# SYSTRAN/faster-whisper

Hardware: AMD Instinct MI355X
Metric: audio-sec/sec (RTF) large-v3 fp16 beam=5 batch=16 (higher is better)
Workload: dtype f16

## Files before the change

faster_whisper_amd/csrc/dec_kernels.hip:

```cpp
#include "common.h"
#include "dec_kernels.h"
#include <stdlib.h>
#include <atomic>
#include <type_traits>

namespace fwd {
static std::atomic<int> g_self_attn_form{0};
static std::atomic<int> g_forms_epoch{0};
static std::atomic<int> g_cross_regs{0};
}

__device__ __forceinline__ size_t frag_off(int row, int k, int KS) {
  return ((size_t)((row >> 4) * KS + (k >> 5)) * 64 + ((k >> 3) & 3) * 16 + (row & 15)) * 8 + (k & 7);
}

__global__ void dec_embed_kernel(const int* __restrict__ tok, const half_t* __restrict__ emb,
                                 const half_t* __restrict__ pos_emb, half_t* __restrict__ x,
                                 half_t* __restrict__ xfrag, int d, const int* __restrict__ d_step, int pos_fixed,
                                 int P, int blk_n) {
  const int r = blockIdx.x;
  const int pos = blk_n > 0 ? pos_fixed + r % blk_n : (pos_fixed >= 0 ? pos_fixed : P - 1 + *d_step);
  const half2_t* e = reinterpret_cast<const half2_t*>(emb + (size_t)tok[r] * d);
  const half2_t* pe = reinterpret_cast<const half2_t*>(pos_emb + (size_t)pos * d);
  half2_t* xo = reinterpret_cast<half2_t*>(x + (size_t)r * d);
// ... 718 lines not shown
    if (LNF) {
      float sa, sb;
      if (SPLIT) {
        sa = xst[a][i][0]; sb = xst[a][i][1];
      } else {
        sa = rs[a]; sb = rq[a];
        sa += __shfl_xor(sa, 16, 64); sa += __shfl_xor(sa, 32, 64);
        sb += __shfl_xor(sb, 16, 64); sb += __shfl_xor(sb, 32, 64);
      }
      mu = sa / (float)K;
      rstd = rsqrtf(fmaxf(sb / (float)K - mu * mu, 0.f) + 1e-5f);
    }
    const int row = (rt0 + a) * 16 + i;
    if (rt0 + a >= n_rt || row >= R) continue;
    const float sx = I8 ? x_scale[row] : 1.f;
    const bool pair_ok = (ldo & 1) == 0;
#pragma unroll
    for (int b = 0; b < NT; ++b) {
      if (ct0 + b >= n_ct) continue;
      const int n = (ct0 + b) * 16 + 4 * g;
      float t4[4];
#pragma unroll
      for (int e = 0; e < 4; ++e) {
        float tv = I8 ? (float)acci[a][b][e] * sx * kws[b][e] : accf[a][b][e];
        if (LNF) tv = rstd * (tv - mu * ks1[b][e]) + kcf[b][e];
        else if (bias) tv += (float)kb[b][e];
        t4[e] = tv;
      }
      if (F32 && pair_ok) {
        float* o = reinterpret_cast<float*>(outv) + (size_t)row * ldo + n;
        if (n + 1 < N) *reinterpret_cast<floatx2*>(o) = floatx2{t4[0], t4[1]};
        else if (n < N) o[0] = t4[0];
        if (n + 3 < N) *reinterpret_cast<floatx2*>(o + 2) = floatx2{t4[2], t4[3]};
        else if (n + 2 < N) o[2] = t4[2];
        continue;
      }
#pragma unroll
      for (int e = 0; e < 4; ++e) {
        if (n + e >= N) continue;
        if (F32) reinterpret_cast<float*>(outv)[(size_t)row * ldo + n + e] = t4[e];
        else reinterpret_cast<half_t*>(outv)[(size_t)row * ldo + n + e] = (half_t)t4[e];
      }
    }
  }
}

#define SA_MAX_CTX 448
static __device__ __forceinline__ float sum8_dpp(float v) {
  v += __builtin_bit_cast(float, __builtin_amdgcn_update_dpp(0, __builtin_bit_cast(int, v), 0xB1, 0xF, 0xF, true));
  v += __builtin_bit_cast(float, __builtin_amdgcn_update_dpp(0, __builtin_bit_cast(int, v), 0x4E, 0xF, 0xF, true));
  v += __builtin_bit_cast(float, __builtin_amdgcn_update_dpp(0, __builtin_bit_cast(int, v), 0x141, 0xF, 0xF, true));
  return v;
}
__global__ __launch_bounds__(1024) __attribute__((amdgpu_waves_per_eu(8, 8))) void dec_self_attn_kernel(const half_t* __restrict__ qkv, int d, half_t* __restrict__ kc,
                                                             half_t* __restrict__ vc, int n_ctx, int cache_ctx,
                                                             int H, const uint8_t* __restrict__ kvidx2, int Kbeam, int kmul,
                                                             half_t* __restrict__ out, const int* __restrict__ d_step,
                                                             int pos_fixed, int P, int R_total, int frag) {
  extern __shared__ float sa_smem[];
  const int lane = threadIdx.x & 63;
  const int wave = __builtin_amdgcn_readfirstlane(threadIdx.x >> 6);
  float* sp = sa_smem + (size_t)wave * 2 * n_ctx;
  int* ssrc = reinterpret_cast<int*>(sp + n_ctx);
  const int h = blockIdx.x, c = blockIdx.y;
  const int r = c * kmul + wave, kb = wave;
  const int step = *d_step;
  const int pos = pos_fixed >= 0 ? pos_fixed : P - 1 + step;
  const int slot = c * Kbeam + kb;
  const int cur = (pos_fixed >= 0) ? 0 : (step & 1);
  const uint8_t* kvidx = kvidx2 + ((size_t)cur * R_total + slot) * n_ctx;
  const half_t* qr = qkv + (size_t)r * 3 * d + h * 64;
  const size_t head_stride = (size_t)cache_ctx * 64;
  const size_t slot_stride = (size_t)H * head_stride;
  const int pg = lane >> 3, cc = lane & 7;
  const half8_t q8 = *reinterpret_cast<const half8_t*>(qr + cc * 8);
  const half8_t kn8 = *reinterpret_cast<const half8_t*>(qr + d + cc * 8);
  const half8_t vn8 = *reinterpret_cast<const half8_t*>(qr + 2 * d + cc * 8);
  float q[8];
#pragma unroll
  for (int e = 0; e < 8; ++e) q[e] = (float)q8[e] * 0.125f;
  if (pg == 0) {
    *reinterpret_cast<half8_t*>(kc + slot * slot_stride + h * head_stride + (size_t)pos * 64 + cc * 8) = kn8;
    *reinterpret_cast<half8_t*>(vc + slot * slot_stride + h * head_stride + (size_t)pos * 64 + cc * 8) = vn8;
  }
  auto dot8 = [&](const half8_t& k) {
    float sacc = 0.f;
#pragma unroll
    for (int e = 0; e < 8; ++e) sacc += q[e] * (float)k[e];
    return sum8_dpp(sacc);
  };
  const float s_new = dot8(kn8);
  float mx = s_new;
  const half_t* kbase = kc + h * head_stride + cc * 8;
  for (int p0 = 0; p0 < pos; p0 += 32) {
    half8_t kv[4];
    int src[4];
#pragma unroll
    for (int j = 0; j < 4; ++j) {
      const int p = p0 + 8 * j + pg;
      const int pc = p < pos ? p : pos - 1;
      src[j] = c * Kbeam + kvidx[pc];
      kv[j] = *reinterpret_cast<const half8_t*>(kbase + src[j] * slot_stride + (size_t)pc * 64);
    }
#pragma unroll
    for (int j = 0; j < 4; ++j) {
      const int p = p0 + 8 * j + pg;
      const float sc = dot8(kv[j]);
      if (p < pos) {
        if (cc == 0) { sp[p] = sc; ssrc[p] = src[j]; }
        mx = fmaxf(mx, sc);
      }
    }
  }
  mx = wave_max(mx);
  __builtin_amdgcn_wave_barrier();
  float sum = 0.f;
  for (int p = lane; p < pos; p += 64) {
    const float e = __expf(sp[p] - mx);
    sp[p] = e;
    sum += e;
  }
  const float e_new = __expf(s_new - mx);
  sum = wave_sum(sum) + e_new;
  __builtin_amdgcn_wave_barrier();
  float acc[8];
#pragma unroll
  for (int e = 0; e < 8; ++e) acc[e] = 0.f;
  const half_t* vb = vc + h * head_stride + cc * 8;
#pragma unroll 4
  for (int p = pg; p < pos; p += 8) {
    const half8_t vv = *reinterpret_cast<const half8_t*>(vb + ssrc[p] * slot_stride + (size_t)p * 64);
    const float w = sp[p];
#pragma unroll
    for (int e = 0; e < 8; ++e) acc[e] += w * (float)vv[e];
  }
#pragma unroll
  for (int e = 0; e < 8; ++e) {
    float a = acc[e];
    a += __shfl_xor(a, 8, 64);
    a += __shfl_xor(a, 16, 64);
    a += __shfl_xor(a, 32, 64);
    acc[e] = a;
  }
  if (pg == 0) {
    const float inv = 1.f / sum;
    half8_t o;
#pragma unroll
    for (int e = 0; e < 8; ++e) o[e] = (half_t)((acc[e] + e_new * (float)vn8[e]) * inv);
    half_t* dst = frag ? out + frag_off(r, h * 64 + cc * 8, d >> 5) : out + (size_t)r * d + h * 64 + cc * 8;
    *reinterpret_cast<half8_t*>(dst) = o;
  }
}

template <int U, bool PIPE, int MAXT, bool PB = false>
__global__ __launch_bounds__(MAXT) void dec_self_attn2_kernel(const half_t* __restrict__ qkv, int d, half_t* __restrict__ kc,
                                                             half_t* __restrict__ vc, int n_ctx, int cache_ctx,
                                                             int H, const uint8_t* __restrict__ kvidx2, int Kbeam, int kmul,
                                                             half_t* __restrict__ out, const int* __restrict__ d_step,
                                                             int pos_fixed, int P, int R_total, int frag) {
  extern __shared__ float sa_smem[];
  constexpr int NB = 4 * U;
  const int lane = threadIdx.x & 63;
  const int wave = __builtin_amdgcn_readfirstlane(threadIdx.x >> 6);
  float* sp = sa_smem + (size_t)wave * 2 * n_ctx;
  int* ssrc = reinterpret_cast<int*>(sp + n_ctx);
  const int h = blockIdx.x, c = blockIdx.y;
  const int r = c * kmul + wave, kb = PB ? 0 : wave;
  const int step = PB ? 0 : *d_step;
  const int pos = PB ? pos_fixed + wave : (pos_fixed >= 0 ? pos_fixed : P - 1 + step);
  const int slot = c * Kbeam + kb;
  const int cur = (pos_fixed >= 0) ? 0 : (step & 1);
  const uint8_t* kvidx = kvidx2 + ((size_t)cur * R_total + slot) * n_ctx;
  const half_t* qr = qkv + (size_t)r * 3 * d + h * 64;
  const size_t head_stride = (size_t)cache_ctx * 64;
  const size_t slot_stride = (size_t)H * head_stride;
  const int pg = lane >> 3, cc = lane & 7;
  for (int p4 = 4 * lane; p4 < pos; p4 += 256) {
    const unsigned w = PB ? 0u : *reinterpret_cast<const unsigned*>(kvidx + p4);
    intx4 s4;
    s4[0] = c * Kbeam + (int)(w & 0xffu); s4[1] = c * Kbeam + (int)((w >> 8) & 0xffu);
    s4[2] = c * Kbeam + (int)((w >> 16) & 0xffu); s4[3] = c * Kbeam + (int)(w >> 24);
    *reinterpret_cast<intx4*>(ssrc + p4) = s4;
  }
  const half8_t q8 = *reinterpret_cast<const half8_t*>(qr + cc * 8);
  const half8_t kn8 = *reinterpret_cast<const half8_t*>(qr + d + cc * 8);
  const half8_t vn8 = *reinterpret_cast<const half8_t*>(qr + 2 * d + cc * 8);
  float q[8];
#pragma unroll
  for (int e = 0; e < 8; ++e) q[e] = (float)q8[e] * 0.125f;
  if (pg == 0) {
    *reinterpret_cast<half8_t*>(kc + slot * slot_stride + h * head_stride + (size_t)pos * 64 + cc * 8) = kn8;
    *reinterpret_cast<half8_t*>(vc + slot * slot_stride + h * head_stride + (size_t)pos * 64 + cc * 8) = vn8;
  }
  auto dot8 = [&](const half8_t& k) {
    float sacc = 0.f;
#pragma unroll
    for (int e = 0; e < 8; ++e) sacc = __builtin_fmaf(q[e], (float)k[e], sacc);
    return sum8_dpp(sacc);
  };
  const float s_new = dot8(kn8);
  float mx = s_new;
  __builtin_amdgcn_wave_barrier();
  const char* kbase = reinterpret_cast<const char*>(kc + h * head_stride);
  const char* vbase = reinterpret_cast<const char*>(vc + h * head_stride);
  const unsigned slot_bytes = (unsigned)(slot_stride * sizeof(half_t));
  struct Batch { half8_t row[NB]; };
  auto fetch = [&](Batch& b, const char* base, int p0, const half_t* sib) {
#pragma unroll
    for (int j = 0; j < NB; ++j) {
      const int p = p0 + 8 * j + pg;
      const int pc = p < pos ? p : pos - 1;
      const unsigned off = (unsigned)ssrc[pc] * slot_bytes + (unsigned)(pc * 128 + cc * 16);
      if (PB && pc >= pos_fixed)
        b.row[j] = *reinterpret_cast<const half8_t*>(sib + (size_t)(pc - pos_fixed) * 3 * d + cc * 8);
      else
        b.row[j] = *reinterpret_cast<const half8_t*>(base + off);
    }
  };
  const half_t* ksib = qkv + (size_t)c * kmul * 3 * d + d + h * 64;
  const half_t* vsib = ksib + d;
  auto score = [&](const Batch& b, int p0) {
#pragma unroll
    for (int j = 0; j < NB; ++j) {
      const int p = p0 + 8 * j + pg;
      const float sc = dot8(b.row[j]);
      if (p < pos) {
        if (cc == 0) sp[p] = sc;
        mx = fmaxf(mx, sc);
      }
    }
  };
  Batch b0, b1;
  if (pos > 0) {
    fetch(b0, kbase, 0, ksib);
    for (int p0 = 0; p0 < pos; p0 += 16 * NB) {
      if (PIPE) {
        fetch(b1, kbase, p0 + 8 * NB, ksib);
        score(b0, p0);
        fetch(b0, kbase, p0 + 16 * NB, ksib);
        score(b1, p0 + 8 * NB);
      } else {
        score(b0, p0);
        if (p0 + 8 * NB < pos) {
          fetch(b0, kbase, p0 + 8 * NB, ksib);
          score(b0, p0 + 8 * NB);
          if (p0 + 16 * NB < pos) fetch(b0, kbase, p0 + 16 * NB, ksib);
        }
      }
    }
    fetch(b0, vbase, 0, vsib);
  }
  mx = wave_max_v(mx);
  __builtin_amdgcn_wave_barrier();
  float sum = 0.f;
  for (int p = lane; p < pos; p += 64) {
    const float e = __expf(sp[p] - mx);
    sp[p] = e;
    sum += e;
  }
  const float e_new = __expf(s_new - mx);
  sum = wave_sum_v(sum) + e_new;
  __builtin_amdgcn_wave_barrier();
  float acc[8];
#pragma unroll
  for (int e = 0; e < 8; ++e) acc[e] = 0.f;
  auto accum = [&](const Batch& b, int p0) {
#pragma unroll
    for (int j = 0; j < NB; ++j) {
      const int p = p0 + 8 * j + pg;
      if (p < pos) {
        const float w = sp[p];
#pragma unroll
        for (int e = 0; e < 8; ++e) acc[e] = __builtin_fmaf(w, (float)b.row[j][e], acc[e]);
      }
    }
  };
  for (int p0 = 0; p0 < pos; p0 += 16 * NB) {
    if (PIPE) {
      fetch(b1, vbase, p0 + 8 * NB, vsib);
      accum(b0, p0);
      fetch(b0, vbase, p0 + 16 * NB, vsib);
      accum(b1, p0 + 8 * NB);
    } else {
      accum(b0, p0);
      if (p0 + 8 * NB < pos) {
        fetch(b0, vbase, p0 + 8 * NB, vsib);
        accum(b0, p0 + 8 * NB);
        if (p0 + 16 * NB < pos) fetch(b0, vbase, p0 + 16 * NB, vsib);
      }
    }
  }
#pragma unroll
  for (int e = 0; e < 8; ++e) acc[e] = sum_x8_x16_x32_v(acc[e]);
  if (pg == 0) {
    const float inv = 1.f / sum;
    half8_t o;
#pragma unroll
    for (int e = 0; e < 8; ++e) o[e] = (half_t)((acc[e] + e_new * (float)vn8[e]) * inv);
    half_t* dst = frag ? out + frag_off(r, h * 64 + cc * 8, d >> 5) : out + (size_t)r * d + h * 64 + cc * 8;
    *reinterpret_cast<half8_t*>(dst) = o;
  }
}

template <int CA_WAVES, bool NTL, int MINW = 1>
__global__ __launch_bounds__(CA_WAVES * 64, MINW) void dec_cross_attn_kernel(const half_t* __restrict__ qx, int d,
                                                             const half_t* __restrict__ ck,
                                                             const half_t* __restrict__ cvt, int T, int kvp,
                                                             int kmul, half_t* __restrict__ out,
                                                             const int* __restrict__ done, int kv_div, int frag,
                                                             const int* __restrict__ slot_map) {
  __shared__ float sm[CA_WAVES][16], sl[CA_WAVES][16];
  __shared__ float so[CA_WAVES][16][65];
  const int h = blockIdx.x, c = blockIdx.y;
  if (done && done[c]) return;
  const int tid = threadIdx.x, lane = tid & 63, wave = tid >> 6;
  const int j = lane & 15, g = lane >> 4;
  const int ce = slot_map[c / kv_div];
  const half_t* kbase = ck + ((size_t)ce * (d >> 6) + h) * kvp * 64 + lane * 8;
  const half_t* vbase = cvt + ((size_t)ce * (d >> 6) + h) * kvp * 64 + lane * 8;
  half8_t qf[2];
  {
    if (j < kmul) {
      const half_t* qp = qx + (size_t)(c * kmul + j) * d + h * 64 + g * 8;
#pragma unroll
      for (int s = 0; s < 2; ++s) {
        half8_t v = *reinterpret_cast<const half8_t*>(qp + s * 32);
#pragma unroll
        for (int e = 0; e < 8; ++e) v[e] = v[e] * (half_t)0.125f;
        qf[s] = v;
      }
    } else {
      qf[0] = half8_t{0, 0, 0, 0, 0, 0, 0, 0};
      qf[1] = qf[0];
    }
  }
  floatx4 o[4];
#pragma unroll
  for (int dt = 0; dt < 4; ++dt) o[dt] = floatx4{0, 0, 0, 0};
  float m_run = -1.0e30f, l_run = 0.f;
  const float LOG2E = 1.4426950408889634f;
  const int ngroups = (T + 31) >> 5;
  auto load_kv = [&](int gi, half8_t (&kf)[4], half8_t (&vf)[4]) {
    const half_t* kp = kbase + (size_t)gi * 2048;
    const half_t* vp = vbase + (size_t)gi * 2048;
#pragma unroll
    for (int q = 0; q < 4; ++q)
      kf[q] = NTL ? __builtin_nontemporal_load(reinterpret_cast<const half8_t*>(kp + q * 512))
                  : *reinterpret_cast<const half8_t*>(kp + q * 512);
#pragma unroll
    for (int dt = 0; dt < 4; ++dt)
      vf[dt] = NTL ? __builtin_nontemporal_load(reinterpret_cast<const half8_t*>(vp + dt * 512))
                   : *reinterpret_cast<const half8_t*>(vp + dt * 512);
  };
  half8_t kcur[4], vcur[4], knxt[4], vnxt[4];
  if (wave < ngroups) load_kv(wave, kcur, vcur);
  for (int gi = wave; gi < ngroups; gi += CA_WAVES) {
    const int base = gi * 32;
    const bool has_next = (gi + CA_WAVES) < ngroups;
    if (has_next) load_kv(gi + CA_WAVES, knxt, vnxt);
    floatx4 s0 = {0, 0, 0, 0}, s1 = {0, 0, 0, 0};
    s0 = __builtin_amdgcn_mfma_f32_16x16x32_f16(kcur[0], qf[0], s0, 0, 0, 0);
    s0 = __builtin_amdgcn_mfma_f32_16x16x32_f16(kcur[1], qf[1], s0, 0, 0, 0);
    s1 = __builtin_amdgcn_mfma_f32_16x16x32_f16(kcur[2], qf[0], s1, 0, 0, 0);
    s1 = __builtin_amdgcn_mfma_f32_16x16x32_f16(kcur[3], qf[1], s1, 0, 0, 0);
    float sc[8];
    float mx = -1.0e30f;
#pragma unroll
    for (int e = 0; e < 8; ++e) {
      float v = (e < 4 ? s0[e] : s1[e - 4]) * LOG2E;
      if (base + 8 * g + e >= T) v = -1.0e30f;
      sc[e] = v;
      mx = fmaxf(mx, v);
    }
    mx = pair16_max(mx);
    mx = pair32_max(mx);
    const float m_new = fmaxf(m_run, mx);
    const float alpha = __builtin_amdgcn_exp2f(m_run - m_new);
    m_run = m_new;
    half8_t pf;
    float psum = 0.f;
#pragma unroll
    for (int e = 0; e < 8; ++e) {
      const float pv = __builtin_amdgcn_exp2f(sc[e] - m_new);
      psum += pv;
      pf[e] = (half_t)pv;
    }
    l_run = l_run * alpha + psum;
#pragma unroll
    for (int dt = 0; dt < 4; ++dt) {
#pragma unroll
      for (int e = 0; e < 4; ++e) o[dt][e] *= alpha;
      o[dt] = __builtin_amdgcn_mfma_f32_16x16x32_f16(vcur[dt], pf, o[dt], 0, 0, 0);
    }
    if (has_next) {
#pragma unroll
      for (int q = 0; q < 4; ++q) { kcur[q] = knxt[q]; vcur[q] = vnxt[q]; }
    }
  }
  l_run = pair16_sum(l_run);
  l_run = pair32_sum(l_run);
  if (g == 0) { sm[wave][j] = m_run; sl[wave][j] = l_run; }
#pragma unroll
  for (int dt = 0; dt < 4; ++dt)
#pragma unroll
    for (int e = 0; e < 4; ++e) so[wave][j][dt * 16 + 4 * g + e] = o[dt][e];
  __syncthreads();
  for (int idx = tid; idx < kmul * 64; idx += CA_WAVES * 64) {
    const int qq = idx >> 6, dh = idx & 63;
    float M = sm[0][qq];
#pragma unroll
    for (int w = 1; w < CA_WAVES; ++w) M = fmaxf(M, sm[w][qq]);
    float Lsum = 0.f, O = 0.f;
#pragma unroll
    for (int w = 0; w < CA_WAVES; ++w) {
      const float f = __builtin_amdgcn_exp2f(sm[w][qq] - M);
      Lsum += sl[w][qq] * f;
      O += so[w][qq][dh] * f;
    }
    const int orow = c * kmul + qq;
    half_t* dst = frag ? out + frag_off(orow, h * 64 + dh, d >> 5) : out + (size_t)orow * d + h * 64 + dh;
    *dst = (half_t)(O / Lsum);
  }
}

__global__ __launch_bounds__(1024) void dec_nospeech_kernel(const float* __restrict__ logits, int V, int row_mul,
                                                            int no_speech_id, float* __restrict__ out) {
  __shared__ float red[32];
  const int b = blockIdx.x;
  const float* lg = logits + (size_t)b * row_mul * V;
  float mx = -3.0e38f;
  for (int v = threadIdx.x; v < V; v += blockDim.x) mx = fmaxf(mx, lg[v]);
  mx = wave_max(mx);
  if ((threadIdx.x & 63) == 0) red[threadIdx.x >> 6] = mx;
  __syncthreads();
  float m2 = -3.0e38f;
  for (int i = 0; i < (int)(blockDim.x >> 6); ++i) m2 = fmaxf(m2, red[i]);
  __syncthreads();
  float s = 0.f;
  for (int v = threadIdx.x; v < V; v += blockDim.x) s += __expf(lg[v] - m2);
  s = wave_sum(s);
  if ((threadIdx.x & 63) == 0) red[threadIdx.x >> 6] = s;
  __syncthreads();
  if (threadIdx.x == 0) {
    float tot = 0.f;
// ... 477 lines not shown
    case 0: frag_variant<4, 2, 2, 5>(st, lnf, xf, Wf, bias, s1, cf, out, R, N, K); break;
    case 1: frag_variant<8, 2, 2, 5>(st, lnf, xf, Wf, bias, s1, cf, out, R, N, K); break;
    case 2: frag_variant<8, 4, 2, 3>(st, lnf, xf, Wf, bias, s1, cf, out, R, N, K); break;
    case 3: frag_variant<8, 4, 2, 4>(st, lnf, xf, Wf, bias, s1, cf, out, R, N, K); break;
    case 4: frag_variant<8, 4, 4, 2>(st, lnf, xf, Wf, bias, s1, cf, out, R, N, K); break;
    case 5: frag_variant<8, 4, 4, 3>(st, lnf, xf, Wf, bias, s1, cf, out, R, N, K); break;
    case 6: frag_variant<4, 4, 2, 3>(st, lnf, xf, Wf, bias, s1, cf, out, R, N, K); break;
    case 7: frag_variant<8, 2, 4, 3>(st, lnf, xf, Wf, bias, s1, cf, out, R, N, K); break;
    case 8: frag_variant<8, 8, 2, 2>(st, lnf, xf, Wf, bias, s1, cf, out, R, N, K); break;
    case 9: frag_variant<4, 4, 4, 2>(st, lnf, xf, Wf, bias, s1, cf, out, R, N, K); break;
    case 23: frag_variant<4, 1, 1, 10>(st, lnf, xf, Wf, bias, s1, cf, out, R, N, K); break;
    case 24: frag_variant<8, 1, 1, 10>(st, lnf, xf, Wf, bias, s1, cf, out, R, N, K); break;
    case 25: frag_variant<4, 1, 2, 6>(st, lnf, xf, Wf, bias, s1, cf, out, R, N, K); break;
    case 26: frag_variant<8, 1, 2, 6>(st, lnf, xf, Wf, bias, s1, cf, out, R, N, K); break;
    case 21: frag_variant<4, 4, 4, 5>(st, lnf, xf, Wf, bias, s1, cf, out, R, N, K); break;
    case 22: frag_variant<8, 4, 4, 5>(st, lnf, xf, Wf, bias, s1, cf, out, R, N, K); break;
    case 10: case 11: case 12:
      return launch_dec_gemm_big(st, variant - 10, xf, Wf, lnf ? nullptr : bias, lnf ? s1 : nullptr, lnf ? cf : nullptr,
                                 nullptr, 0, out, N, nullptr, R, N, K, 0);
    default: return -1;
  }
  return 0;
}

static int dec_linear_role(int N, int K) { return N == 3 * K ? 0 : (N >= 2560 ? 2 : (K >= 2560 ? 3 : 1)); }
struct DecBigRule { int rows; int cfg; };
static const DecBigRule DEC_BIG_RULES[4][2] = {
     {{640, 2}, {1280, 0}},
     {{1088, 1}, {1 << 30, 1}},
     {{512, 2}, {1280, 0}},
     {{832, 1}, {1 << 30, 1}},
};
static int dec_big_cfg_for(int R, int N, int K) {
  const DecBigRule* r = DEC_BIG_RULES[dec_linear_role(N, K)];
  if (R >= r[1].rows) return r[1].cfg;
  if (R >= r[0].rows) return r[0].cfg;
  return -1;
}
#define DEC_BIG_MIN_ROWS_I8 1024
int dec_big_min_rows_of(int role, int compute_type) {
  if (compute_type == 1) return DEC_BIG_MIN_ROWS_I8;
  if (role >= 0 && role < 4) return DEC_BIG_RULES[role][0].rows;
  int lo = DEC_BIG_RULES[0][0].rows;
  for (int k = 1; k < 4; ++k) lo = DEC_BIG_RULES[k][0].rows < lo ? DEC_BIG_RULES[k][0].rows : lo;
  return lo;
}

static bool skinny_one_tile(int R, int N) { return R <= 16 || (R <= 96 && N <= 1280); }

int launch_dec_gemm_frag(hipStream_t st, const half_t* xf, const half_t* Wf, const half_t* bias, const float* s1,
                         const float* cf, const half_t* res, int ldr, half_t* out, int ldo, half_t* out_frag, int R,
                         int N, int K, int act) {
  const int cfg = dec_big_cfg_for(R, N, K);
  if (cfg >= 0 &&
      launch_dec_gemm_big(st, cfg, xf, Wf, bias, s1, cf, res, ldr, out, ldo, out_frag, R, N, K, act) == 0)
    return 0;
  return launch_dec_gemm_skinny(st, xf, Wf, bias, s1, cf, res, ldr, out, ldo, out_frag, R, N, K, act);
}

int dec_big_min_rows() { return dec_big_min_rows_of(-1, 0); }

int launch_dec_gemm_skinny(hipStream_t st, const half_t* xf, const half_t* Wf, const half_t* bias, const float* s1,
                           const float* cf, const half_t* res, int ldr, half_t* out, int ldo, half_t* out_frag, int R,
                           int N, int K, int act) {
  if (K % 32 != 0 || N % 32 != 0 || R < 1) return -1;
  const int waves = K >= 2560 ? 8 : 4;
  const bool one_tile = skinny_one_tile(R, N);
  if (one_tile) {
    if (s1) frag_go<true, 1, 1, 10>(st, waves, xf, Wf, bias, s1, cf, res, ldr, out, ldo, out_frag, R, N, K, act);
    else frag_go<false, 1, 1, 10>(st, waves, xf, Wf, bias, s1, cf, res, ldr, out, ldo, out_frag, R, N, K, act);
    return 0;
  }
  if (s1) frag_go<true, 2, 2>(st, waves, xf, Wf, bias, s1, cf, res, ldr, out, ldo, out_frag, R, N, K, act);
  else frag_go<false, 2, 2>(st, waves, xf, Wf, bias, s1, cf, res, ldr, out, ldo, out_frag, R, N, K, act);
  return 0;
}

int launch_dec_gemm_skinny_tiles(hipStream_t st, int tiles, const half_t* xf, const half_t* Wf, const half_t* bias,
                                 const float* s1, const float* cf, const half_t* res, int ldr, half_t* out, int ldo,
                                 half_t* out_frag, int R, int N, int K, int act) {
  if (K % 32 != 0 || N % 32 != 0 || R < 1) return -1;
  const int waves = K >= 2560 ? 8 : 4;
  if (tiles == 1) {
    if (s1) frag_go<true, 1, 1, 10>(st, waves, xf, Wf, bias, s1, cf, res, ldr, out, ldo, out_frag, R, N, K, act);
    else frag_go<false, 1, 1, 10>(st, waves, xf, Wf, bias, s1, cf, res, ldr, out, ldo, out_frag, R, N, K, act);
  } else if (tiles == 2) {
    if (s1) frag_go<true, 2, 2>(st, waves, xf, Wf, bias, s1, cf, res, ldr, out, ldo, out_frag, R, N, K, act);
    else frag_go<false, 2, 2>(st, waves, xf, Wf, bias, s1, cf, res, ldr, out, ldo, out_frag, R, N, K, act);
  } else {
    return -1;
  }
  return 0;
}

int launch_dec_gemm_frag_i8(hipStream_t st, const int8_t* xq, const float* x_scale, const int8_t* Wq,
                            const float* w_scale, const half_t* bias, const half_t* res, int ldr, half_t* out, int ldo,
                            int R, int N, int K, int act) {
  if (K % 64 != 0 || N % 32 != 0 || R < 1 || !x_scale || !w_scale) return -1;
  if (R >= DEC_BIG_MIN_ROWS_I8 && N % 64 == 0) {
    const dim3 g4(N / 64, ((R + 15) / 16 + 3) / 4);
    if (K >= 2560)
      dec_gemm_frag_i8_kernel<8, 4, 4, 3><<<g4, 512, 0, st>>>(xq, x_scale, Wq, w_scale, bias, res, ldr, out, ldo, R, N, K, act);
    else
      dec_gemm_frag_i8_kernel<4, 4, 4, 5><<<g4, 256, 0, st>>>(xq, x_scale, Wq, w_scale, bias, res, ldr, out, ldo, R, N, K, act);
    return 0;
  }
  const dim3 grid(N / 32, ((R + 15) / 16 + 1) / 2);
  if (K >= 2560)
    dec_gemm_frag_i8_kernel<8, 2, 2><<<grid, 512, 0, st>>>(xq, x_scale, Wq, w_scale, bias, res, ldr, out, ldo, R, N, K, act);
  else
    dec_gemm_frag_i8_kernel<4, 2, 2><<<grid, 256, 0, st>>>(xq, x_scale, Wq, w_scale, bias, res, ldr, out, ldo, R, N, K, act);
  return 0;
}

template <bool I8, bool LNF, int RT>
static void wave_go(hipStream_t st, const void* xf, const float* x_scale, const void* Wf, const float* w_scale,
                    const float* s1, const float* cf, float* out, int ldo, int R, int N, int K) {
  constexpr int NT = 2, WM = 1, WN = 4;
  const int n_rt = (R + 15) / 16, n_ct = (N + 15) / 16;
  const int n_cg = ((n_ct + NT * WN - 1) / (NT * WN) + 7) & ~7;
  const int n_rg = (n_rt + RT * WM - 1) / (RT * WM);
  dec_gemm_wave_kernel<I8, LNF, true, RT, NT, WM, WN><<<n_cg * n_rg, WM * WN * 64, 0, st>>>(
      xf, x_scale, Wf, w_scale, nullptr, s1, cf, out, ldo, R, N, K, n_rg);
}

int launch_dec_logits(hipStream_t st, bool i8, const void* xf, const float* x_scale, const void* Wf,
                      const float* w_scale, const float* s1, const float* cf, float* out, int ldo, int R, int N, int K) {
  if (K % (i8 ? 64 : 32) != 0 || R < 1) return -1;
  if (i8 ? (!x_scale || !w_scale) : ((s1 == nullptr) != (cf == nullptr))) return -1;
  const int n_rt = (R + 15) / 16;
#define WG(RT)                                                                                   \
  do {                                                                                           \
    if (i8) wave_go<true, false, RT>(st, xf, x_scale, Wf, w_scale, s1, cf, out, ldo, R, N, K);   \
    else if (s1) wave_go<false, true, RT>(st, xf, x_scale, Wf, w_scale, s1, cf, out, ldo, R, N, K); \
    else wave_go<false, false, RT>(st, xf, x_scale, Wf, w_scale, s1, cf, out, ldo, R, N, K);     \
  } while (0)
  if (n_rt == 1) WG(1);
  else if (n_rt == 2) WG(2);
  else if (n_rt == 3) WG(3);
  else if (n_rt == 4) WG(4);
  else WG(5);
#undef WG
  return 0;
}

bool self_attn_block_ok(int n_ctx, int cache_ctx, int d, int R_total) {
  return (n_ctx & 3) == 0 && (size_t)R_total * cache_ctx * d * sizeof(half_t) < ((size_t)1 << 32);
}

void launch_self_attn(hipStream_t st, const half_t* qkv, int d, half_t* kc, half_t* vc, int n_ctx, int cache_ctx, int H,
                      const uint8_t* kvidx2, int Kbeam, int kmul, half_t* out, int rows, const int* d_step,
                      int pos_fixed, int P, int R_total, int frag, int blk_n) {
  if (blk_n > 0) {
    dec_self_attn2_kernel<1, true, 1024, true><<<dim3(H, rows / blk_n), blk_n * 64, (size_t)blk_n * 2 * n_ctx * sizeof(float), st>>>(
        qkv, d, kc, vc, n_ctx, cache_ctx, H, kvidx2, Kbeam, blk_n, out, d_step, pos_fixed, P, R_total, frag);
    return;
  }
  const dim3 grid(H, rows / kmul);
  const size_t lds = (size_t)kmul * 2 * n_ctx * sizeof(float);
  int form = g_self_attn_form.load(std::memory_order_relaxed);
  if ((n_ctx & 3) != 0 || (size_t)R_total * cache_ctx * d * sizeof(half_t) >= ((size_t)1 << 32)) form = 1;
  if (form == 0) form = (kmul <= 8 && (int)(grid.x * grid.y) <= 768) ? 2 : 3;
  if (form == 2 && kmul > 8) form = 3;
#define SA_ARGS qkv, d, kc, vc, n_ctx, cache_ctx, H, kvidx2, Kbeam, kmul, out, d_step, pos_fixed, P, R_total, frag
  if (form == 1) dec_self_attn_kernel<<<grid, kmul * 64, lds, st>>>(SA_ARGS);
  else if (form == 2) dec_self_attn2_kernel<4, false, 512><<<grid, kmul * 64, lds, st>>>(SA_ARGS);
  else dec_self_attn2_kernel<1, true, 1024><<<grid, kmul * 64, lds, st>>>(SA_ARGS);
#undef SA_ARGS
}
void set_self_attn_form(int form) { g_self_attn_form.store(form); g_forms_epoch.fetch_add(1); }
int kernel_forms_epoch() { return g_forms_epoch.load(); }
void bump_kernel_forms_epoch() { g_forms_epoch.fetch_add(1); }

void launch_cross_attn(hipStream_t st, const half_t* qx, int d, const half_t* ck, const half_t* cvt, int T, int kvp,
                       int kmul, half_t* out, int B, int H, const int* done, int kv_div, int frag, const int* slot_map) {
  const int cap = g_cross_regs.load(std::memory_order_relaxed);
  if (cap == 1)
    dec_cross_attn_kernel<8, true, 5><<<dim3(H, B), 512, 0, st>>>(qx, d, ck, cvt, T, kvp, kmul, out, done, kv_div, frag, slot_map);
  else if (cap == 2)
    dec_cross_attn_kernel<8, true, 6><<<dim3(H, B), 512, 0, st>>>(qx, d, ck, cvt, T, kvp, kmul, out, done, kv_div, frag, slot_map);
  else
    dec_cross_attn_kernel<8, true><<<dim3(H, B), 512, 0, st>>>(qx, d, ck, cvt, T, kvp, kmul, out, done, kv_div, frag, slot_map);
}
void set_cross_attn_regs(int cap) { g_cross_regs.store(cap); g_forms_epoch.fetch_add(1); }

void launch_nospeech(hipStream_t st, const float* logits, int V, int row_mul, int no_speech_id, float* out, int B) {
  dec_nospeech_kernel<<<B, 1024, 0, st>>>(logits, V, row_mul, no_speech_id, out);
}

void launch_logits_process(hipStream_t st, const GenDev& gp, float* logits, const unsigned long long* sup_bits,
                           const int* hist2, const float* cum2, const int* d_step, const int* done, float* cand_val,
                           int* cand_tok) {
  const bool wide = gp.ts_begin >= 48 * LP_THREADS;
#define LP_GO(SMP, TXI) \
  dec_logits_process_kernel<SMP, TXI><<<gp.R, LP_THREADS, 0, st>>>(gp, logits, sup_bits, hist2, cum2, d_step, done, cand_val, cand_tok)
  if (gp.sample) { if (wide) LP_GO(true, 48); else LP_GO(true, 0); }
  else { if (wide) LP_GO(false, 48); else LP_GO(false, 0); }
#undef LP_GO
}

void launch_beam_update(hipStream_t st, const GenDev& gp, const float* cand_val, const int* cand_tok, int* hist2,
                        float* cum2, uint8_t* kvidx2, int* cur_tok, const int* d_step, int* done, int* n_done,
                        int* n_fin, int* fin_tok, int* fin_len, float* fin_score, float* fin_cum) {
  dec_beam_update_kernel<<<gp.B, 64, 0, st>>>(gp, cand_val, cand_tok, hist2, cum2, kvidx2, cur_tok, d_step, done,
                                              n_done, n_fin, fin_tok, fin_len, fin_score, fin_cum);
}

void launch_step_advance(hipStream_t st, int* d_step) { dec_step_advance_kernel<<<1, 1, 0, st>>>(d_step); }

void launch_token_prob(hipStream_t st, const float* logits, int V, const int* target, float* out, int out_stride,
                       int out_off, int rows, int row_mul) {
  dec_token_prob_kernel<<<rows, 1024, 0, st>>>(logits, V, target, out, out_stride, out_off, row_mul);
}

void launch_cross_probs(hipStream_t st, const half_t* qx, int d, const half_t* ck, int T, int kvp, const int* heads,
                        int n_layer_heads, int n_sel, float* probs, int n_tok, int tok_idx, int B, int blk_n) {
  const int bn = blk_n > 0 ? blk_n : 1;
  dec_cross_probs_kernel<<<dim3(n_layer_heads, B * bn), 256, 0, st>>>(qx, d, ck, T, kvp, heads, n_sel, probs, n_tok,
                                                                      tok_idx, bn);
}

}
```

Before: 3190.

## Use buffer loads, precomputed byte offsets and inline fma_mix in decoder self-attention

The self-attention decode kernel now stores precomputed byte offsets per cache position in LDS instead of slot indices, and fetches K/V rows with raw buffer loads from a scalar buffer resource. The LDS arrays are padded to a whole batch, so tail fetches need no clamping. Score and weighted-accumulate steps are hand-written inline assembly using v_fma_mix_f32 with DPP reductions. The loops are restructured so full batches skip bounds checks, with sched_barriers to keep loads ahead of compute. This cuts address arithmetic and conversion instructions in a memory-bound loop, at the cost of fragile inline asm, slightly larger LDS and a 32-bit offset range.

Result: faster. 3225, median of 5 (+1.1%).

```diff
diff --git a/faster_whisper_amd/csrc/dec_kernels.hip b/faster_whisper_amd/csrc/dec_kernels.hip
--- a/faster_whisper_amd/csrc/dec_kernels.hip
+++ b/faster_whisper_amd/csrc/dec_kernels.hip
@@ -894,6 +894,79 @@
   }
 }
 
+struct SaFull { static constexpr bool full = true; };
+struct SaPart { static constexpr bool full = false; };
+static __host__ __device__ __forceinline__ int sa_lds_ctx(int n_ctx, int batch) { return (n_ctx + batch - 1) / batch * batch; }
+static __device__ __forceinline__ float max_finite(float a, float b) {
+  return __builtin_amdgcn_fmed3f(a, b, __builtin_inff());
+}
+static __device__ __forceinline__ void score4(float (&sc)[4], const float (&q)[8], const half8_t& k0, const half8_t& k1,
+                                              const half8_t& k2, const half8_t& k3) {
+  const intx4 a = __builtin_bit_cast(intx4, k0), b = __builtin_bit_cast(intx4, k1), c = __builtin_bit_cast(intx4, k2),
+              d = __builtin_bit_cast(intx4, k3);
+  asm(
+      "v_fma_mix_f32 %0, %4, %12, 0 op_sel_hi:[0,1,0]\n\t"
+      "v_fma_mix_f32 %1, %4, %16, 0 op_sel_hi:[0,1,0]\n\t"
+      "v_fma_mix_f32 %2, %4, %20, 0 op_sel_hi:[0,1,0]\n\t"
+      "v_fma_mix_f32 %3, %4, %24, 0 op_sel_hi:[0,1,0]\n\t"
+      "v_fma_mix_f32 %0, %5, %12, %0 op_sel:[0,1,0] op_sel_hi:[0,1,0]\n\t"
+      "v_fma_mix_f32 %1, %5, %16, %1 op_sel:[0,1,0] op_sel_hi:[0,1,0]\n\t"
+      "v_fma_mix_f32 %2, %5, %20, %2 op_sel:[0,1,0] op_sel_hi:[0,1,0]\n\t"
+      "v_fma_mix_f32 %3, %5, %24, %3 op_sel:[0,1,0] op_sel_hi:[0,1,0]\n\t"
+      "v_fma_mix_f32 %0, %6, %13, %0 op_sel_hi:[0,1,0]\n\t"
+      "v_fma_mix_f32 %1, %6, %17, %1 op_sel_hi:[0,1,0]\n\t"
+      "v_fma_mix_f32 %2, %6, %21, %2 op_sel_hi:[0,1,0]\n\t"
+      "v_fma_mix_f32 %3, %6, %25, %3 op_sel_hi:[0,1,0]\n\t"
+      "v_fma_mix_f32 %0, %7, %13, %0 op_sel:[0,1,0] op_sel_hi:[0,1,0]\n\t"
+      "v_fma_mix_f32 %1, %7, %17, %1 op_sel:[0,1,0] op_sel_hi:[0,1,0]\n\t"
+      "v_fma_mix_f32 %2, %7, %21, %2 op_sel:[0,1,0] op_sel_hi:[0,1,0]\n\t"
+      "v_fma_mix_f32 %3, %7, %25, %3 op_sel:[0,1,0] op_sel_hi:[0,1,0]\n\t"
+      "v_fma_mix_f32 %0, %8, %14, %0 op_sel_hi:[0,1,0]\n\t"
+      "v_fma_mix_f32 %1, %8, %18, %1 op_sel_hi:[0,1,0]\n\t"
+      "v_fma_mix_f32 %2, %8, %22, %2 op_sel_hi:[0,1,0]\n\t"
+      "v_fma_mix_f32 %3, %8, %26, %3 op_sel_hi:[0,1,0]\n\t"
+      "v_fma_mix_f32 %0, %9, %14, %0 op_sel:[0,1,0] op_sel_hi:[0,1,0]\n\t"
+      "v_fma_mix_f32 %1, %9, %18, %1 op_sel:[0,1,0] op_sel_hi:[0,1,0]\n\t"
+      "v_fma_mix_f32 %2, %9, %22, %2 op_sel:[0,1,0] op_sel_hi:[0,1,0]\n\t"
+      "v_fma_mix_f32 %3, %9, %26, %3 op_sel:[0,1,0] op_sel_hi:[0,1,0]\n\t"
+      "v_fma_mix_f32 %0, %10, %15, %0 op_sel_hi:[0,1,0]\n\t"
+      "v_fma_mix_f32 %1, %10, %19, %1 op_sel_hi:[0,1,0]\n\t"
+      "v_fma_mix_f32 %2, %10, %23, %2 op_sel_hi:[0,1,0]\n\t"
+      "v_fma_mix_f32 %3, %10, %27, %3 op_sel_hi:[0,1,0]\n\t"
+      "v_fma_mix_f32 %0, %11, %15, %0 op_sel:[0,1,0] op_sel_hi:[0,1,0]\n\t"
+      "v_fma_mix_f32 %1, %11, %19, %1 op_sel:[0,1,0] op_sel_hi:[0,1,0]\n\t"
+      "v_fma_mix_f32 %2, %11, %23, %2 op_sel:[0,1,0] op_sel_hi:[0,1,0]\n\t"
+      "v_fma_mix_f32 %3, %11, %27, %3 op_sel:[0,1,0] op_sel_hi:[0,1,0]\n\t"
+      "v_add_f32_dpp %0, %0, %0 quad_perm:[1,0,3,2] row_mask:0xf bank_mask:0xf bound_ctrl:1\n\t"
+      "v_add_f32_dpp %1, %1, %1 quad_perm:[1,0,3,2] row_mask:0xf bank_mask:0xf bound_ctrl:1\n\t"
+      "v_add_f32_dpp %2, %2, %2 quad_perm:[1,0,3,2] row_mask:0xf bank_mask:0xf bound_ctrl:1\n\t"
+      "v_add_f32_dpp %3, %3, %3 quad_perm:[1,0,3,2] row_mask:0xf bank_mask:0xf bound_ctrl:1\n\t"
+      "v_add_f32_dpp %0, %0, %0 quad_perm:[2,3,0,1] row_mask:0xf bank_mask:0xf bound_ctrl:1\n\t"
+      "v_add_f32_dpp %1, %1, %1 quad_perm:[2,3,0,1] row_mask:0xf bank_mask:0xf bound_ctrl:1\n\t"
+      "v_add_f32_dpp %2, %2, %2 quad_perm:[2,3,0,1] row_mask:0xf bank_mask:0xf bound_ctrl:1\n\t"
+      "v_add_f32_dpp %3, %3, %3 quad_perm:[2,3,0,1] row_mask:0xf bank_mask:0xf bound_ctrl:1\n\t"
+      "v_add_f32_dpp %0, %0, %0 row_half_mirror row_mask:0xf bank_mask:0xf bound_ctrl:1\n\t"
+      "v_add_f32_dpp %1, %1, %1 row_half_mirror row_mask:0xf bank_mask:0xf bound_ctrl:1\n\t"
+      "v_add_f32_dpp %2, %2, %2 row_half_mirror row_mask:0xf bank_mask:0xf bound_ctrl:1\n\t"
+      "v_add_f32_dpp %3, %3, %3 row_half_mirror row_mask:0xf bank_mask:0xf bound_ctrl:1"
+      : "=&v"(sc[0]), "=&v"(sc[1]), "=&v"(sc[2]), "=&v"(sc[3])
+      : "v"(q[0]), "v"(q[1]), "v"(q[2]), "v"(q[3]), "v"(q[4]), "v"(q[5]), "v"(q[6]), "v"(q[7]),
+        "v"(a[0]), "v"(a[1]), "v"(a[2]), "v"(a[3]), "v"(b[0]), "v"(b[1]), "v"(b[2]), "v"(b[3]),
+        "v"(c[0]), "v"(c[1]), "v"(c[2]), "v"(c[3]), "v"(d[0]), "v"(d[1]), "v"(d[2]), "v"(d[3]));
+}
+static __device__ __forceinline__ void fma_row(float (&acc)[8], float w, const half8_t& v) {
+  const intx4 r = __builtin_bit_cast(intx4, v);
+  asm("v_fma_mix_f32 %0, %8, %9, %0 op_sel_hi:[0,1,0]\n\t"
+      "v_fma_mix_f32 %1, %8, %9, %1 op_sel:[0,1,0] op_sel_hi:[0,1,0]\n\t"
+      "v_fma_mix_f32 %2, %8, %10, %2 op_sel_hi:[0,1,0]\n\t"
+      "v_fma_mix_f32 %3, %8, %10, %3 op_sel:[0,1,0] op_sel_hi:[0,1,0]\n\t"
+      "v_fma_mix_f32 %4, %8, %11, %4 op_sel_hi:[0,1,0]\n\t"
+      "v_fma_mix_f32 %5, %8, %11, %5 op_sel:[0,1,0] op_sel_hi:[0,1,0]\n\t"
+      "v_fma_mix_f32 %6, %8, %12, %6 op_sel_hi:[0,1,0]\n\t"
+      "v_fma_mix_f32 %7, %8, %12, %7 op_sel:[0,1,0] op_sel_hi:[0,1,0]"
+      : "+v"(acc[0]), "+v"(acc[1]), "+v"(acc[2]), "+v"(acc[3]), "+v"(acc[4]), "+v"(acc[5]), "+v"(acc[6]), "+v"(acc[7])
+      : "v"(w), "v"(r[0]), "v"(r[1]), "v"(r[2]), "v"(r[3]));
+}
 template <int U, bool PIPE, int MAXT, bool PB = false>
 __global__ __launch_bounds__(MAXT) void dec_self_attn2_kernel(const half_t* __restrict__ qkv, int d, half_t* __restrict__ kc,
                                                              half_t* __restrict__ vc, int n_ctx, int cache_ctx,
@@ -902,10 +975,12 @@
                                                              int pos_fixed, int P, int R_total, int frag) {
   extern __shared__ float sa_smem[];
   constexpr int NB = 4 * U;
+  constexpr int BP = 8 * NB;
   const int lane = threadIdx.x & 63;
   const int wave = __builtin_amdgcn_readfirstlane(threadIdx.x >> 6);
-  float* sp = sa_smem + (size_t)wave * 2 * n_ctx;
-  int* ssrc = reinterpret_cast<int*>(sp + n_ctx);
+  const int npad = sa_lds_ctx(n_ctx, BP);
+  float* sp = sa_smem + (size_t)wave * 2 * npad;
+  unsigned* soff = reinterpret_cast<unsigned*>(sp + npad);
   const int h = blockIdx.x, c = blockIdx.y;
   const int r = c * kmul + wave, kb = PB ? 0 : wave;
   const int step = PB ? 0 : *d_step;
@@ -916,13 +991,19 @@
   const half_t* qr = qkv + (size_t)r * 3 * d + h * 64;
   const size_t head_stride = (size_t)cache_ctx * 64;
   const size_t slot_stride = (size_t)H * head_stride;
+  const unsigned slot_bytes = (unsigned)(slot_stride * sizeof(half_t));
   const int pg = lane >> 3, cc = lane & 7;
   for (int p4 = 4 * lane; p4 < pos; p4 += 256) {
     const unsigned w = PB ? 0u : *reinterpret_cast<const unsigned*>(kvidx + p4);
+    const unsigned o = (unsigned)(c * Kbeam) * slot_bytes + (unsigned)p4 * 128u;
     intx4 s4;
-    s4[0] = c * Kbeam + (int)(w & 0xffu); s4[1] = c * Kbeam + (int)((w >> 8) & 0xffu);
-    s4[2] = c * Kbeam + (int)((w >> 16) & 0xffu); s4[3] = c * Kbeam + (int)(w >> 24);
-    *reinterpret_cast<intx4*>(ssrc + p4) = s4;
+    s4[0] = (int)(o + (w & 0xffu) * slot_bytes); s4[1] = (int)(o + 128u + ((w >> 8) & 0xffu) * slot_bytes);
+    s4[2] = (int)(o + 256u + ((w >> 16) & 0xffu) * slot_bytes); s4[3] = (int)(o + 384u + (w >> 24) * slot_bytes);
+    *reinterpret_cast<intx4*>(soff + p4) = s4;
+  }
+  if (!PB && pos > 0 && pos % BP != 0) {
+    const unsigned last = (unsigned)(c * Kbeam + kvidx[pos - 1]) * slot_bytes + (unsigned)(pos - 1) * 128u;
+    for (int p = pos + lane; p < (pos + BP - 1) / BP * BP; p += 64) soff[p] = last;
   }
   const half8_t q8 = *reinterpret_cast<const half8_t*>(qr + cc * 8);
   const half8_t kn8 = *reinterpret_cast<const half8_t*>(qr + d + cc * 8);
@@ -943,54 +1024,74 @@
   const float s_new = dot8(kn8);
   float mx = s_new;
   __builtin_amdgcn_wave_barrier();
-  const char* kbase = reinterpret_cast<const char*>(kc + h * head_stride);
-  const char* vbase = reinterpret_cast<const char*>(vc + h * head_stride);
-  const unsigned slot_bytes = (unsigned)(slot_stride * sizeof(half_t));
+  auto plane = [&](const half_t* cache) {
+    const uintptr_t a = reinterpret_cast<uintptr_t>(cache + h * head_stride);
+    const unsigned lo = __builtin_amdgcn_readfirstlane((unsigned)a), hi = __builtin_amdgcn_readfirstlane((unsigned)(a >> 32));
+    const unsigned bytes = __builtin_amdgcn_readfirstlane((unsigned)R_total * slot_bytes - (unsigned)(h * head_stride * sizeof(half_t)));
+    return __builtin_amdgcn_make_buffer_rsrc(reinterpret_cast<void*>(((uintptr_t)hi << 32) | lo), 0, (int)bytes, 0x00020000);
+  };
+  const __amdgpu_buffer_rsrc_t kplane = plane(kc), vplane = plane(vc);
+  const unsigned cc16 = (unsigned)cc * 16u;
   struct Batch { half8_t row[NB]; };
-  auto fetch = [&](Batch& b, const char* base, int p0, const half_t* sib) {
+  auto fetch = [&](Batch& b, __amdgpu_buffer_rsrc_t pl, int p0, const half_t* sib) {
 #pragma unroll
     for (int j = 0; j < NB; ++j) {
       const int p = p0 + 8 * j + pg;
-      const int pc = p < pos ? p : pos - 1;
-      const unsigned off = (unsigned)ssrc[pc] * slot_bytes + (unsigned)(pc * 128 + cc * 16);
+      const int pc = (!PB || p < pos) ? p : pos - 1;
       if (PB && pc >= pos_fixed)
         b.row[j] = *reinterpret_cast<const half8_t*>(sib + (size_t)(pc - pos_fixed) * 3 * d + cc * 8);
       else
-        b.row[j] = *reinterpret_cast<const half8_t*>(base + off);
+        b.row[j] = __builtin_bit_cast(half8_t, __builtin_amdgcn_raw_buffer_load_b128(pl, (int)(soff[pc] + cc16), 0, 0));
     }
   };
   const half_t* ksib = qkv + (size_t)c * kmul * 3 * d + d + h * 64;
   const half_t* vsib = ksib + d;
   auto score = [&](const Batch& b, int p0) {
-#pragma unroll
-    for (int j = 0; j < NB; ++j) {
-      const int p = p0 + 8 * j + pg;
-      const float sc = dot8(b.row[j]);
-      if (p < pos) {
-        if (cc == 0) sp[p] = sc;
-        mx = fmaxf(mx, sc);
-      }
+    float sc[NB];
+#pragma unroll
+    for (int j = 0; j < NB; j += 4) {
+      float s4[4];
+      score4(s4, q, b.row[j], b.row[j + 1], b.row[j + 2], b.row[j + 3]);
+#pragma unroll
+      for (int i = 0; i < 4; ++i) {
+        sc[j + i] = s4[i];
+        mx = max_finite(mx, s4[i]);
+      }
+    }
+    if (cc == 0) {
+#pragma unroll
+      for (int j = 0; j < NB; ++j) sp[p0 + 8 * j + pg] = sc[j];
     }
   };
   Batch b0, b1;
   if (pos > 0) {
-    fetch(b0, kbase, 0, ksib);
-    for (int p0 = 0; p0 < pos; p0 += 16 * NB) {
-      if (PIPE) {
-        fetch(b1, kbase, p0 + 8 * NB, ksib);
+    int p0 = 0;
+    fetch(b0, kplane, 0, ksib);
+    if (PIPE) {
+      for (; p0 + 2 * BP < pos; p0 += 2 * BP) {
+        fetch(b1, kplane, p0 + BP, ksib);
+        __builtin_amdgcn_sched_barrier(0);
         score(b0, p0);
-        fetch(b0, kbase, p0 + 16 * NB, ksib);
-        score(b1, p0 + 8 * NB);
+        fetch(b0, kplane, p0 + 2 * BP, ksib);
+        __builtin_amdgcn_sched_barrier(0);
+        score(b1, p0 + BP);
+      }
+      if (p0 + BP < pos) {
+        fetch(b1, kplane, p0 + BP, ksib);
+        __builtin_amdgcn_sched_barrier(0);
+        score(b0, p0);
+        score(b1, p0 + BP);
       } else {
         score(b0, p0);
-        if (p0 + 8 * NB < pos) {
-          fetch(b0, kbase, p0 + 8 * NB, ksib);
-          score(b0, p0 + 8 * NB);
-          if (p0 + 16 * NB < pos) fetch(b0, kbase, p0 + 16 * NB, ksib);
-        }
-      }
-    }
-    fetch(b0, vbase, 0, vsib);
+      }
+    } else {
+      for (; p0 + BP < pos; p0 += BP) {
+        score(b0, p0);
+        fetch(b0, kplane, p0 + BP, ksib);
+      }
+      score(b0, p0);
+    }
+    fetch(b0, vplane, 0, vsib);
   }
   mx = wave_max_v(mx);
   __builtin_amdgcn_wave_barrier();
@@ -1006,32 +1107,43 @@
   float acc[8];
 #pragma unroll
   for (int e = 0; e < 8; ++e) acc[e] = 0.f;
-  auto accum = [&](const Batch& b, int p0) {
+  auto accum = [&](const Batch& b, int p0, auto kind) {
 #pragma unroll
     for (int j = 0; j < NB; ++j) {
       const int p = p0 + 8 * j + pg;
-      if (p < pos) {
-        const float w = sp[p];
-#pragma unroll
-        for (int e = 0; e < 8; ++e) acc[e] = __builtin_fmaf(w, (float)b.row[j][e], acc[e]);
+      if (decltype(kind)::full || p < pos) {
+        fma_row(acc, sp[p], b.row[j]);
       }
     }
   };
-  for (int p0 = 0; p0 < pos; p0 += 16 * NB) {
+  if (pos > 0) {
+    int p0 = 0;
     if (PIPE) {
-      fetch(b1, vbase, p0 + 8 * NB, vsib);
-      accum(b0, p0);
-      fetch(b0, vbase, p0 + 16 * NB, vsib);
-      accum(b1, p0 + 8 * NB);
+      for (; p0 + 2 * BP < pos; p0 += 2 * BP) {
+        fetch(b1, vplane, p0 + BP, vsib);
+        __builtin_amdgcn_sched_barrier(0);
+        accum(b0, p0, SaFull{});
+        fetch(b0, vplane, p0 + 2 * BP, vsib);
+        __builtin_amdgcn_sched_barrier(0);
+        accum(b1, p0 + BP, SaFull{});
+      }
+      if (p0 + BP < pos) {
+        fetch(b1, vplane, p0 + BP, vsib);
+        __builtin_amdgcn_sched_barrier(0);
+        accum(b0, p0, SaFull{});
+        accum(b1, p0 + BP, SaPart{});
+      } else {
+        accum(b0, p0, SaPart{});
+      }
     } else {
-      accum(b0, p0);
-      if (p0 + 8 * NB < pos) {
-        fetch(b0, vbase, p0 + 8 * NB, vsib);
-        accum(b0, p0 + 8 * NB);
-        if (p0 + 16 * NB < pos) fetch(b0, vbase, p0 + 16 * NB, vsib);
-      }
-    }
-  }
+      for (; p0 + BP < pos; p0 += BP) {
+        accum(b0, p0, SaFull{});
+        fetch(b0, vplane, p0 + BP, vsib);
+      }
+      accum(b0, p0, SaPart{});
+    }
+  }
+  asm volatile("s_nop 1" : "+v"(acc[0]), "+v"(acc[1]), "+v"(acc[2]), "+v"(acc[3]), "+v"(acc[4]), "+v"(acc[5]), "+v"(acc[6]), "+v"(acc[7]));
 #pragma unroll
   for (int e = 0; e < 8; ++e) acc[e] = sum_x8_x16_x32_v(acc[e]);
   if (pg == 0) {
@@ -1815,16 +1927,16 @@
                       const uint8_t* kvidx2, int Kbeam, int kmul, half_t* out, int rows, const int* d_step,
                       int pos_fixed, int P, int R_total, int frag, int blk_n) {
   if (blk_n > 0) {
-    dec_self_attn2_kernel<1, true, 1024, true><<<dim3(H, rows / blk_n), blk_n * 64, (size_t)blk_n * 2 * n_ctx * sizeof(float), st>>>(
+    dec_self_attn2_kernel<1, true, 1024, true><<<dim3(H, rows / blk_n), blk_n * 64, (size_t)blk_n * 2 * sa_lds_ctx(n_ctx, 32) * sizeof(float), st>>>(
         qkv, d, kc, vc, n_ctx, cache_ctx, H, kvidx2, Kbeam, blk_n, out, d_step, pos_fixed, P, R_total, frag);
     return;
   }
   const dim3 grid(H, rows / kmul);
-  const size_t lds = (size_t)kmul * 2 * n_ctx * sizeof(float);
   int form = g_self_attn_form.load(std::memory_order_relaxed);
   if ((n_ctx & 3) != 0 || (size_t)R_total * cache_ctx * d * sizeof(half_t) >= ((size_t)1 << 32)) form = 1;
   if (form == 0) form = (kmul <= 8 && (int)(grid.x * grid.y) <= 768) ? 2 : 3;
   if (form == 2 && kmul > 8) form = 3;
+  const size_t lds = (size_t)kmul * 2 * (form == 1 ? n_ctx : sa_lds_ctx(n_ctx, form == 2 ? 128 : 32)) * sizeof(float);
 #define SA_ARGS qkv, d, kc, vc, n_ctx, cache_ctx, H, kvidx2, Kbeam, kmul, out, d_step, pos_fixed, P, R_total, frag
   if (form == 1) dec_self_attn_kernel<<<grid, kmul * 64, lds, st>>>(SA_ARGS);
   else if (form == 2) dec_self_attn2_kernel<4, false, 512><<<grid, kmul * 64, lds, st>>>(SA_ARGS);
```
